# optimusride/altro-cpp

Hardware: AMD Instinct MI355X
Metric: trajectories solved/sec (AL-iLQR to tol), unicycle 101 knots, batched (higher is better)
Workload: dtype f64; 1 GPU; BASELINE configs[2]: batch 4096/GPU unicycle kTurn90 (n=3, m=2, 101 knots), goal + control-bound constraints, full AL loop, default SolverOptions; batch_per_gpu=4096, global_batch=4096, knot_points=101, parallelism=instance-sharded x1 (no data-path collective; RCCL all_gather of result records), device=AMD Radeon Graphics, cus=256

## Files before the change

### altro-cpp_amd/csrc/altro_engine.hpp

```cpp
#pragma once

#include <algorithm>
#include <atomic>
#include <chrono>
#include <cmath>
#include <cstdio>
#include <cstdlib>
#include <cstring>
#include <limits>
#include <map>
#include <string>
#include <thread>
#include <type_traits>
#include <vector>

#include "altro_kernels.hpp"
#include "altro_problem.hpp"

namespace altro_hip {

#define ALTRO_HIP_CHECK(expr)                                                                  \
  do {                                                                                         \
    hipError_t e_ = (expr);                                                                    \
    if (e_ != hipSuccess) {                                                                    \
// ... 1 lines not shown
      snprintf(buf_, sizeof(buf_), "%s:%d: %s -> %s", __FILE__, __LINE__, #expr,               \
               hipGetErrorString(e_));                                                         \
      err_ = buf_;                                                                             \
      return ALTRO_HIP_ERROR;                                                                  \
    }                                                                                          \
  } while (0)

#define ALTRO_TRY(expr)                  \
  do {                                   \
    altro_status st_ = (expr);           \
    if (st_ != ALTRO_OK) return st_;     \
  } while (0)

constexpr int kSpecAuto = -1;
enum FwdSrcSwitch { kFwdSrcAuto = -1, kFwdSrcOther = 0, kFwdSrcGlobal = 1 };
struct Switches {
  struct OptInt {
    bool set = false;
    int v = 0;
  };
  bool poison_on = false;
  unsigned poison_pattern = 0;
  int poison_mix = 0;
  OptInt persist_at;
  bool twin = true;
  bool segments = true;
  OptInt chains;
  OptInt fwd_per_wave;
  int fwd_src = kFwdSrcAuto;
  int sweep_loop = -1;
  OptInt loop_per_cu;
  int cand_front = 6;
  bool twin_debug = false;
  int twin_depth = kTwinDefaultDepth;
  int twin_misclaim = 0;
  const char* sweep_log = nullptr;
  bool loop_log = false;
  bool force_valu_backward = false, force_coop_backward = false;
  bool dense_expansions = true;
  int spec_mode = kSpecAuto;
  bool fast_forward = false;
  bool begin_merged = true;
  bool no_fused = false;

  static bool NotZero(const char* e) { return !(e && atoi(e) == 0); }
  static bool Is(const char* e, const char* what) { return e && std::strcmp(e, what) == 0; }
  Switches() {
    auto env = [](const char* name) { return std::getenv(name); };
    auto number = [&](const char* name) {
      const char* e = env(name);
      return e ? OptInt{true, atoi(e)} : OptInt{};
    };
    if (const char* e = env("ALTRO_HIP_DEBUG_POISON")) {
      poison_on = true;
      poison_pattern = (unsigned)strtoul(e, nullptr, 16);
      poison_mix = std::strchr(e, ',') != nullptr;
    }
    persist_at = number("ALTRO_HIP_PERSIST_AT");
    twin = NotZero(env("ALTRO_HIP_TWIN"));
    segments = NotZero(env("ALTRO_HIP_SEGMENTS"));
    chains = number("ALTRO_HIP_CHAINS");
    if (chains.set) chains.v = std::max(1, std::min(kMaxSweepChains, chains.v));
    fwd_per_wave = number("ALTRO_HIP_FWD_PER_WAVE");
    if (const char* e = env("ALTRO_HIP_FWD_SRC")) fwd_src = Is(e, "global") ? kFwdSrcGlobal : kFwdSrcOther;
    if (const char* e = env("ALTRO_HIP_SWEEP_LOOP")) sweep_loop = NotZero(e) ? 1 : 0;
    loop_per_cu = number("ALTRO_HIP_LOOP_PER_CU");
    if (const char* e = env("ALTRO_HIP_CAND_FRONT")) cand_front = std::max(0, std::min(kLineSearchLanes - 1, atoi(e)));
    twin_debug = env("ALTRO_HIP_TWIN_DEBUG") != nullptr;
    if (const char* e = env("ALTRO_HIP_TWIN_DEPTH")) twin_depth = std::max(1, std::min(kTwinMaxDepth, atoi(e)));
    if (const char* e = env("ALTRO_HIP_TWIN_MISCLAIM")) twin_misclaim = std::max(0, atoi(e));
    sweep_log = env("ALTRO_HIP_SWEEP_LOG");
    loop_log = env("ALTRO_HIP_LOOP_LOG") != nullptr;
    force_valu_backward = Is(env("ALTRO_HIP_BACKWARD"), "valu");
    force_coop_backward = Is(env("ALTRO_HIP_BACKWARD"), "coop");
    dense_expansions = env("ALTRO_HIP_NO_DENSE_EXPANSIONS") == nullptr;
    const char* spec = env("ALTRO_HIP_SPECULATION");
    spec_mode = Is(spec, "off") ? (int)kSpecOff : Is(spec, "free") ? (int)kSpecFree : Is(spec, "wave") ? (int)kSpecWave : kSpecAuto;
    fast_forward = env("ALTRO_HIP_FAST_FORWARD_STALLS") != nullptr;
    begin_merged = !Is(env("ALTRO_HIP_BEGIN_SOLVE"), "split");
    no_fused = env("ALTRO_HIP_NO_FUSED_SWEEP") != nullptr;
  }
};

inline DevOpts ToDevOpts(const altro_options& o) {
  DevOpts d{};
  d.max_iterations_total = o.max_iterations_total;
  d.max_iterations_outer = o.max_iterations_outer;
  d.max_iterations_inner = o.max_iterations_inner;
  d.bp_reg_fail_threshold = o.bp_reg_fail_threshold;
  d.check_forwardpass_bounds = o.check_forwardpass_bounds;
  d.line_search_max_iterations = o.line_search_max_iterations;
  d.reset_duals = o.reset_duals;
  d.cost_tolerance = o.cost_tolerance;
  d.gradient_tolerance = o.gradient_tolerance;
  d.bp_reg_increase_factor = o.bp_reg_increase_factor;
  d.bp_reg_initial = o.bp_reg_initial;
  d.bp_reg_max = o.bp_reg_max;
  d.bp_reg_min = o.bp_reg_min;
  d.state_max = o.state_max;
  d.control_max = o.control_max;
  d.line_search_lower_bound = o.line_search_lower_bound;
  d.line_search_upper_bound = o.line_search_upper_bound;
// ... 1401 lines not shown
  altro_status SetTrajectoryImpl(const ProblemSpec& s) {
    if (!uploaded_) return ALTRO_OK;
    ALTRO_HIP_CHECK(hipSetDevice(desc_.device_id));
    ALTRO_TRY(Sync());
    const double* Xh = !s.has_X ? nullptr : (s.X_view ? s.X_view : s.X.data());
    const double* Uh = !s.has_U ? nullptr : (s.U_view ? s.U_view : s.U.data());
    ALTRO_TRY(UploadRec(A_.X, N_ + 1, R::nP, n, Xh, s.traj_per_instance != 0));
    ALTRO_TRY(UploadRec(A_.U, N_, R::mP, m, Uh, s.traj_per_instance != 0));
    ALTRO_HIP_CHECK(CopySync(X_init_, A_.X, (size_t)(N_ + 1) * R::nP * Bp_ * sizeof(T), hipMemcpyDeviceToDevice));
    ALTRO_HIP_CHECK(CopySync(U_init_, A_.U, (size_t)N_ * R::mP * Bp_ * sizeof(T), hipMemcpyDeviceToDevice));
    return ALTRO_OK;
  }

  altro_status CheckKnotModels(const ProblemSpec& s) {
    for (size_t k = 0; k < s.knot_model.size() && (int)k < desc_.N; ++k) {
      const int w = s.knot_model[k];
      if (w < 0 || w >= kModelCount) {
        err_ = "altro_set_knot_models: knot " + std::to_string(k) + " asks for model " + std::to_string(w) + ", this handle's model " +
               (kModelCount > 1 ? "source lists " + std::to_string(kModelCount) + " models (ALTRO_USER_MODELS)"
                                : std::string("is a single model (a user source with #define ALTRO_USER_MODELS A, B, ... holds several)"));
        return ALTRO_INVALID_ARG;
      }
    }
    return ALTRO_OK;
  }
  size_t ExpBytes(size_t columns) const { return ((size_t)kBwdFrontPad + (size_t)N_ + 2) * RR::EP * columns * sizeof(RS); }
  void SizeShadowColumns() {
    B_ = desc_.batch;
    N_ = desc_.N;
    Bp_ = ((B_ + kBlock - 1) / kBlock) * kBlock;
    twin_cap_ = 0;
    if constexpr (kMfmaBackward) {
      if (sw_.twin && !sw_.fast_forward && !sw_.no_fused) {
        const int want = std::min({Bp_, 16384, ((persist_at_ * 3 / 2 + 8 + kBlock - 1) / kBlock) * kBlock});
        if (ExpBytes((size_t)(Bp_ + want)) < (size_t)0xffffffffu) twin_cap_ = want;
      }
    }
    seg_total_ = 0;
    seg_col0_ = Bp_;
    if constexpr (kMfmaBackward) {
      if (sw_.segments && !sw_.fast_forward && B_ > persist_at_) {
        const int want = (Bp_ * 5 / 8) / kBlock * kBlock;
        if (ExpBytes((size_t)(Bp_ + want + twin_cap_)) < (size_t)0xffffffffu) seg_total_ = want;
      }
    }
    seg_parts_ = 4;
    Bp_ += seg_total_ + twin_cap_;
  }
  static UserTypeTable UserTypes() {
    UserTypeTable t;
    for (int i = 0; i < UserCostList::size; ++i) t.cost_nparams.push_back(UserCostParams(i));
    for (int i = 0; i < UserConList::size; ++i) {
      int np = -1, p = -1, eq = -1;
      UserConInfo(i, &np, &p, &eq);
      t.con_nparams.push_back(np);
      t.con_p.push_back(p);
      t.con_eq.push_back(eq);
    }
    return t;
  }
  altro_status AdoptProblem(const CompiledProblem<T>& cp) {
    if (cp.status != ALTRO_OK) {
      err_ = cp.err;
      return cp.status;
    }
    pd_ = cp.pd;
    knot_class_ = cp.knot_class;
// ... 820 lines not shown
        A.act_list = d_loop_tail_;
        A.act_count = d_loop_ctl_ + kLwTail;
      } else if (whole_batch) {
        A.act_list = nullptr;
        A.act_count = nullptr;
        A.act_count_const = B_;
      } else if (lists.n == 1) {
        A.act_list = lists.list[0];
        A.act_count = lists.count[0];
      } else {
        int* const merged_count = d_counter_ + (size_t)C * r.cstride;
        hipLaunchKernelGGL((k_merge_lists<0>), dim3(1), dim3(256), 0, stream_, lists, d_merged_, merged_count);
        A.act_list = d_merged_;
        A.act_count = merged_count;
        timing_.launches += 1;
      }
      A.host_count = nullptr;
      A.next_list = nullptr;
      A.next_count = nullptr;
      PoisonLds();
      if (r.prof) {
        r.fused_ev = r.nev;
        hipEventRecord(ProfEvent(r.nev++), stream_);
      }
      bool circles = false;
      for (int k = 0; k < pd_.nruns; ++k)
        circles = circles || pd_.runs[k].fast == kFastC || pd_.runs[k].fast == kFastCB || pd_.runs[k].fast == kFastBC;
      int* const out = r.loop_launched ? d_loop_ctl_ + kLwWords : d_counter_ + r.max_sweeps + 2;
      const int spec = sw_.spec_mode == kSpecAuto ? (circles ? (int)kSpecWave : (int)kSpecFree) : sw_.spec_mode;
      TwinCtl tw{};
      if (twin_cap_ > 0 && !A.hist && !r.d.fast_forward_stalls) {
        if (!twin_box_clean_)
          hipMemsetAsync(d_twin_box_, 0, TwinBoxWords() * sizeof(unsigned long long), stream_);
        const int pool = std::min(twin_cap_, std::max(ninst, num_cus_ - ninst));
        tw = TwinCtl{d_twin_box_, d_twin_box_ + (size_t)2 * twin_cap_ * kTwWords, ninst, twin_cap_, Bp_ - twin_cap_, kTwinLag, sw_.twin_debug ? 1 : 0,
                     pool, any_split ? 1 : sw_.twin_depth, sw_.twin_misclaim};
      }
      const dim3 g(ninst + (tw.base > 0 ? tw.npool : 0)), b3(kFwdWaves * kBlock), b4((kFwdWaves + 1) * kBlock);
      timing_.twin_workgroups = tw.base > 0 ? (int)g.x - ninst : 0;
      ForEachFusedVariant([&](auto v) {
        using V = decltype(v);
        if (V::circles == circles && V::spec == spec && V::segments == any_split)
          hipLaunchKernelGGL((k_sweep_fused<T, M, V::circles, V::spec, V::segments>), g, V::spec == kSpecOff ? b3 : b4, fused_lds_bytes_,
                             stream_, A, d_pd_, pd_, r.d, r.mode, 1, out, tw);
      });
      if (r.prof) hipEventRecord(ProfEvent(r.nev++), stream_);
      r.persistent_launched = true;
      timing_.launches += 1;
    }
    return ALTRO_OK;
  }
  altro_status WaitForDevice(SolveRun& r) {
    if (r.nap_ok && !r.nap)
      r.nap = r.loop_launched || std::chrono::duration<double, std::micro>(std::chrono::steady_clock::now() - r.t0).count() > kHostNapAfterUs;
    if (r.nap && tail_ev_) {
      ALTRO_HIP_CHECK(hipEventRecord(tail_ev_, stream_));
      for (;;) {
        const hipError_t q = hipEventQuery(tail_ev_);
        if (q == hipSuccess) break;
        if (q != hipErrorNotReady) ALTRO_HIP_CHECK(q);
        std::this_thread::sleep_for(std::chrono::microseconds(20));
        timing_.host_naps += 1;
      }
    }
    for (int c = 1; c < r.C; ++c) ALTRO_HIP_CHECK(hipStreamSynchronize(r.chain[c].st));
    ALTRO_HIP_CHECK(hipStreamSynchronize(stream_));
    ALTRO_HIP_CHECK(hipGetLastError());
    return ALTRO_OK;
  }
// ... 45 lines not shown
      }
      if (twin_cap_ > 0 && sw_.twin_debug) ALTRO_TRY(DumpTwinMailboxes());
      if (extra[kRwSyncErr] != 0) {
        err_ = "k_sweep_fused: a forward wave gave up waiting for its sequence word (software synchronisation)";
        return ALTRO_HIP_ERROR;
      }
      timing_.fused_sweeps = extra[kRwChainLoops];
      timing_.fused_instance_iterations = extra[kRwUnits];
      sweeps = std::max(sweeps, extra[kRwSweeps]);
    }
    timing_.sweeps = sweeps;
    return ALTRO_OK;
  }
  size_t TwinBoxWords() const { return (size_t)2 * twin_cap_ * (kTwWords + 1); }
  altro_status DumpTwinMailboxes() {
    const int nbox = 2 * twin_cap_;
    std::vector<unsigned long long> box((size_t)nbox * kTwWords);
    ALTRO_HIP_CHECK(CopySync(box.data(), d_twin_box_, box.size() * sizeof(unsigned long long), hipMemcpyDeviceToHost));
    int hist[4] = {0, 0, 0, 0}, why[8] = {0}, by_depth[kTwinMaxDepth + 2] = {0};
    unsigned long long t0 = ~0ull;
    for (int s = 0; s < twin_cap_; ++s)
      if (box[(size_t)s * kTwWords + kTwStamp + kTsPStart]) t0 = std::min(t0, box[(size_t)s * kTwWords + kTwStamp + kTsPStart]);
    auto us_of = [&](const unsigned long long* ts, int i) { return ts[i] ? (double)(long long)(ts[i] - t0) * 0.01 : -1.0; };
    int shown = 0;
    double last_commit = 0, last_pend = 0, last_tstart = 0, last_leave = 0;
    int s_commit = -1, s_pend = -1;
    for (int s = 0; s < nbox; ++s) {
      const unsigned long long* w = &box[(size_t)s * kTwWords];
      const unsigned long long* ts = w + kTwStamp;
      auto us = [&](int i) { return us_of(ts, i); };
      if (s >= twin_cap_ && w[kTwClaim] != 0) {
        hist[w[kTwHand] & 3]++;
        by_depth[std::min<unsigned long long>(w[kTwGen], kTwinMaxDepth + 1)]++;
        const int limit = timing_.twin_claims <= 48 ? 1 : 8;
        if ((shown++ % limit) == 0)
          fprintf(stderr, "  segment %4d depth %d inst %d from %d: it %d..%d hand %d | start %.0f go %.0f cloned %.0f first %.0f snap %.0f claimed %.0f "
                  "done %.0f (loops %llu) verdict %.0f handed %.0f commit %.0f\n", s, (int)w[kTwGen], (int)w[kTwInst] - 1, (int)w[kTwPred] - 1,
                  (int)(w[kTwClaim] >> 32), (int)w[kTwEnd], (int)(w[kTwHand] & 3), us(kTsTStart), us(kTsTGo), us(kTsTCloned), us(kTsTFirst), us(kTsPSnap),
                  us(kTsPClaim), us(kTsTDone), ts[kTsTLoops], us(kTsTVerdict), us(kTsPHand), us(kTsTCommit));
      }
      if (w[kTwWhy] != 0) {
        why[w[kTwWhy] & 7]++;
        if (why[w[kTwWhy] & 7] <= 3)
          fprintf(stderr, "  worker %d refused its successor: why %d at it_inner %d (claim start %d)\n", s, (int)(w[kTwWhy] & 7),
                  (int)((w[kTwWhy] >> 8) & 0xffff), (int)((w[kTwWhy] >> 24) & 0xffff));
      }
      if (us(kTsTCommit) > last_commit) { last_commit = us(kTsTCommit); s_commit = s; }
      if (us(kTsPEnd) > last_pend) { last_pend = us(kTsPEnd); s_pend = s; }
      last_leave = std::max(last_leave, us(kTsPHand));
      last_tstart = std::max(last_tstart, us(kTsTStart));
    }
    fprintf(stderr, "twin timeline: last commit %.0f us (mailbox %d), last primary that finished by itself %.0f us (slot %d), last hand-over %.0f us, "
            "last pool start %.0f us\n", last_commit, s_commit, last_pend, s_pend, last_leave, last_tstart);
    fprintf(stderr, "twin mailboxes: pool %d claims %d confirmed joints %d | segments by depth: 1: %d 2: %d 3: %d 4: %d 5: %d | hand word: open %d ok %d refused %d "
            "revoked %d | refusals: streak broke %d, passed %d, counters %d, rho %d, drho %d, break since snapshot %d\n", (int)timing_.twin_workgroups,
            (int)timing_.twin_claims, (int)timing_.twin_handovers, by_depth[1], by_depth[2], by_depth[3], by_depth[4], by_depth[5], hist[0], hist[1], hist[2],
            hist[3], why[1], why[2], why[3], why[4], why[5], why[6]);
    return ALTRO_OK;
  }
  void AccountProfile(SolveRun& r) {
    float ms = 0, fused_ms = 0;
    hipEventElapsedTime(&ms, prof_ev_[0], prof_ev_[1]);
    timing_.init_ms = ms;
    for (int c = 0; c < r.C; ++c) {
      const std::vector<size_t>& ev = r.chain[c].ev;
      for (size_t e0 = 0; e0 + 3 < ev.size(); e0 += 3) {
        hipEventElapsedTime(&ms, prof_ev_[ev[e0]], prof_ev_[ev[e0 + 1]]);
        timing_.expansions_ms += ms;
        hipEventElapsedTime(&ms, prof_ev_[ev[e0 + 1]], prof_ev_[ev[e0 + 2]]);
        timing_.backward_pass_ms += ms;
        hipEventElapsedTime(&ms, prof_ev_[ev[e0 + 2]], prof_ev_[ev[e0 + 3]]);
        timing_.forward_pass_ms += ms;
      }
// ... 154 lines not shown
```

### altro-cpp_amd/csrc/altro_kernels.hpp

```cpp
#pragma once

#include <type_traits>

#include "altro_device.hpp"

namespace altro_hip {

constexpr int kFwdWaves = 3;
constexpr int kEAheadToErrWord = -7;
constexpr int kFwdSpinLimit = 1 << 22;
template <int kDummy>
__global__ __launch_bounds__(256) void k_poison_columns(unsigned* arr, unsigned rows, unsigned Bp, unsigned col0, unsigned ncols,
                                                         unsigned words, unsigned pattern, int mix) {
  const size_t per_row = (size_t)ncols * words, total = (size_t)rows * per_row;
  for (size_t i = (size_t)blockIdx.x * 256 + threadIdx.x; i < total; i += (size_t)gridDim.x * 256) {
    const size_t r = i / per_row, w = i - r * per_row;
    arr[(r * Bp + col0) * words + w] = mix ? (pattern ^ ((unsigned)i * 2654435761u)) : pattern;
  }
}
template <int kDummy>
__global__ __launch_bounds__(256) void k_poison_lds(unsigned pattern, int words, int mix, int* sink) {
  extern __shared__ unsigned poison_smem[];
  for (int i = threadIdx.x; i < words; i += 256) poison_smem[i] = mix ? (pattern ^ ((unsigned)i * 2654435761u)) : pattern;
  __syncthreads();
// ... 3202 lines not shown
      load_rec<T, R::nP>(sX + k * R::nP, xr);
#pragma unroll
      for (int i = 0; i < R::mP; ++i) ur[i] = T(0);
      if (k < N) load_rec<T, R::mP>(sU + k * R::mP, ur);
      T E[R::EP];
#pragma unroll
      for (int e = 0; e < R::EP; ++e) E[e] = T(0);
      const T J = knot_cost_expansion<T, n, m>(C, pd, kc, rb, xr, ur, E + R::oLx, E + R::oLu, E + R::oLxx, E + R::oLxu,
                                               E + R::oLuu);
      A.costs[(unsigned)k * Bp + (unsigned)b] = J;
      sCost[k] = J;
      if (k < N) discrete_jacobian<T, M>(xr, ur, T(pd->hstep), E + R::oAB);
      using RS = rec_scalar_t<T, M>;
      using RR = Rec<RS, n, m>;
      store_rec_as<T, RS, R::EP, RR::EP, R::eE>(RECP((RS*)A.EXP, k, RR::EP), E);
    }
    toff = (toff + ((cnt + kBlock - 1) / kBlock) * kBlock) % nthreads;
  }
}

enum SpecMode { kSpecOff = 0, kSpecWave = 1, kSpecFree = 3 };
ALTRO_DEV constexpr bool spec_has_wave4(int spec) { return spec == kSpecWave || spec == kSpecFree; }

struct TwinCtl {
  unsigned long long* box;
  unsigned long long* state;
  int base;
  int cap;
  int col0;
  int lag;
  int debug;
  int npool;
  int depth;
  int misclaim;
};
enum TwinStamp { kTsPStart = 0, kTsPSnap = 1, kTsPClaim = 2, kTsPHand = 3, kTsPLoopsAtSnap = 4, kTsTStart = 5, kTsTGo = 6, kTsTCloned = 7,
                 kTsTFirst = 8, kTsTDone = 9, kTsTVerdict = 10, kTsTCommit = 11, kTsTLoops = 12, kTsPEnd = 13 };
enum TwinWord {
  kTwSeq = 0,
  kTwSnap = 1,
  kTwProg = 7,
  kTwSucc = 8,
  kTwEnd = 9,
  kTwGen = 10,
  kTwInst = 11,
  kTwClaim = 12,
  kTwClaimRho = 13,
  kTwClaimDrho = 14,
  kTwClaimSnap = 15,
  kTwHand = 16,
  kTwHandLoops = 17,
  kTwWhy = 18,
  kTwPred = 19,
  kTwStamp = 20,
  kTwWords = 40
};
constexpr unsigned long long kTwOk = 1, kTwRefused = 2, kTwRevoked = 3;
constexpr unsigned long long kTwSuccId = 0xffffull;
constexpr unsigned long long kTwFrozen = 1ull << 32;
constexpr unsigned long long kTwsSnap = 1, kTwsClosed = 2, kTwsLocked = 4, kTwsFull = 8, kTwsBusy = 16;
#ifndef ALTRO_TWIN_DEPTH
#define ALTRO_TWIN_DEPTH 3
#endif
constexpr int kTwinDefaultDepth = ALTRO_TWIN_DEPTH;
constexpr int kTwinMaxDepth = 5;
constexpr int kTwinMinRemaining = 12;
#ifndef ALTRO_TWIN_LAG
#define ALTRO_TWIN_LAG 1
#endif
constexpr int kTwinLag = ALTRO_TWIN_LAG;
constexpr int kTwinIdlePolls = 1 << 15;
constexpr int kTwinHandPolls = 1 << 16;
ALTRO_DEV unsigned long long tw_load(const unsigned long long* p) {
  return __hip_atomic_load(p, __ATOMIC_RELAXED, __HIP_MEMORY_SCOPE_AGENT);
}
ALTRO_DEV void tw_store(unsigned long long* p, unsigned long long v) {
  __hip_atomic_store(p, v, __ATOMIC_RELAXED, __HIP_MEMORY_SCOPE_AGENT);
}
ALTRO_DEV void tw_order() { asm volatile("s_waitcnt vmcnt(0)" ::: "memory"); }
ALTRO_DEV bool tw_cas(unsigned long long* p, unsigned long long expect, unsigned long long v) {
  return __hip_atomic_compare_exchange_strong(p, &expect, v, __ATOMIC_RELAXED, __ATOMIC_RELAXED, __HIP_MEMORY_SCOPE_AGENT);
}
ALTRO_DEV unsigned long long tw_bits(double x) { return (unsigned long long)__double_as_longlong(x); }
ALTRO_DEV double tw_dbl(unsigned long long x) { return __longlong_as_double((long long)x); }
ALTRO_DEV int tw_remaining(const DevOpts& o, unsigned long long prog, int end_inner) {
  const int it_in = (int)(prog >> 32), it_tot = (int)(prog & 0xffffffffull);
  if (end_inner > 0) return end_inner - it_in;
  const int r1 = o.max_iterations_inner - it_in, r2 = o.max_iterations_total - it_tot;
  return r1 < r2 ? r1 : r2;
}
ALTRO_DEV int tw_keep(int R, int lag) { return (R + lag) / 2 + 1; }
ALTRO_DEV bool tw_claimable(int R, int lag) { return R >= 2 * kTwinMinRemaining && R - tw_keep(R, lag) >= kTwinMinRemaining; }
ALTRO_DEV void tw_cancel_chain(const TwinCtl& tw, unsigned long long* box) {
  unsigned long long nx = __hip_atomic_fetch_or(box + kTwSucc, kTwFrozen, __ATOMIC_RELAXED, __HIP_MEMORY_SCOPE_AGENT) & kTwSuccId;
  for (int guard = 0; nx != 0 && nx <= (unsigned long long)(2 * tw.cap) && guard < (2 << kTwinMaxDepth); ++guard) {
    const int id = (int)nx - 1;
    unsigned long long* sb = tw.box + (size_t)id * kTwWords;
    nx = __hip_atomic_fetch_or(sb + kTwSucc, kTwFrozen, __ATOMIC_RELAXED, __HIP_MEMORY_SCOPE_AGENT) & kTwSuccId;
    tw_cas(sb + kTwHand, 0ull, kTwRefused);
    __hip_atomic_fetch_or(tw.state + id, kTwsClosed, __ATOMIC_RELAXED, __HIP_MEMORY_SCOPE_AGENT);
  }
}

template <class T>
struct TailCtx {
  const DevArrays<T>& A;
  const ProblemDesc* pd;
  const DevOpts& o;
  const TwinCtl& tw;
  int* sweeps_out;
  double* ff;
  int tid;
};
struct TwinWorker {
  unsigned long long* box = nullptr;
  int slot = -1;
  bool is_twin = false;
  int streak = 0;
  int break_total = -1;
  unsigned long long ver = 0;
  bool closed = false;
  bool shown = false;
  unsigned long long succ = 0, claim = 0;
  unsigned long long peek = 0;
  bool full = false;
  bool confirmed = false;
  int loops0 = 0;
  ALTRO_DEV void stamp(const TwinCtl& tw, int which, long long value = -1) const {
    if (box && tw.debug) tw_store(box + kTwStamp + which, (unsigned long long)(value >= 0 ? value : wall_clock64()));
  }
  ALTRO_DEV void close(const TwinCtl& tw) const {
    __hip_atomic_fetch_or(tw.state + slot, kTwsClosed, __ATOMIC_RELAXED, __HIP_MEMORY_SCOPE_AGENT);
  }
};

template <class T, bool SEG, bool SOFT>
ALTRO_DEV void fused_report(const TailCtx<T>& C, int b_real, const int* sync_words, int chain_loops, int units, int skipped) {
  const DevArrays<T>& A = C.A;
  int* const sweeps_out = C.sweeps_out;
  if (sweeps_out && C.tid == 0) {
    atomicMax(sweeps_out + kRwChainLoops, chain_loops);
    atomicAdd(sweeps_out + kRwUnits, units);
    atomicMax(sweeps_out + kRwGroupLoops, units + skipped);
    int chain = 0;
    if (A.chain_size) {
      chain = (SEG && A.seg_end && b_real >= A.B && A.seg_hi > 0 && b_real >= A.seg_lo) ? (b_real - A.seg_lo) / A.seg_hi : b_real / A.chain_size;
      chain = chain < kMaxSweepChains - 1 ? chain : kMaxSweepChains - 1;
    }
    atomicMax(sweeps_out + kRwSweeps, A.chain_base[chain] + chain_loops);
    if (SOFT && sync_words[kSyErr] != 0) atomicMax(sweeps_out + kRwSyncErr, 1);
  }
}

ALTRO_DEV int tw_scan(const TwinCtl& tw, const DevOpts& o, int nsl, int nall, int self, int lane, int* waiting_out) {
  int waiting = 0, key = 0;
  for (int v0 = 0; v0 < nall; v0 += kBlock) {
    const int v = v0 + lane;
    bool open = false;
    if (v < nall) {
      const int id = v < nsl ? v : tw.cap + (v - nsl);
      const unsigned long long st = id == self ? kTwsClosed : tw_load(tw.state + id);
      open = (st & (kTwsClosed | kTwsFull)) == 0 && (v < nsl || (st & kTwsBusy) != 0);
      if (open && (st & kTwsSnap) != 0) {
        const unsigned long long* bx = tw.box + (size_t)id * kTwWords;
        const int R = tw_remaining(o, tw_load(bx + kTwProg), (int)tw_load(bx + kTwEnd));
        open = tw_claimable(R, tw.lag);
        if (open && (st & kTwsLocked) == 0) {
          const int k2 = ((R < 0x7fff ? R : 0x7fff) << 16) | (0xffff - (v & 0xffff));
          key = k2 > key ? k2 : key;
        }
      }
    }
    waiting += __popcll(__ballot(open));
  }
  for (int d = 32; d > 0; d >>= 1) {
    const int other = __shfl_xor(key, d);
    key = other > key ? other : key;
  }
  *waiting_out = waiting;
  return key;
}
template <class T>
ALTRO_DEV int tw_try_claim(const TailCtx<T>& C, int v, int nsl, int self) {
  const TwinCtl& tw = C.tw;
  const DevOpts& o = C.o;
  int* const sweeps_out = C.sweeps_out;
  double* const ff = C.ff;
  int got = 0;
  const int id = v < nsl ? v : tw.cap + (v - nsl);
  unsigned long long* bx = tw.box + (size_t)id * kTwWords;
  const unsigned long long st0 = kTwsSnap | (v < nsl ? 0ull : kTwsBusy);
  if (!tw_cas(tw.state + id, st0, st0 | kTwsLocked)) return 0;
  unsigned long long more = 0;
  const unsigned long long ver = tw_load(bx + kTwSeq);
  if (ver != 0) {
    const unsigned long long* buf = bx + kTwSnap + 3 * (ver & 1);
    const unsigned long long c0 = tw_load(buf), rb = tw_load(buf + 1), db = tw_load(buf + 2);
    const unsigned long long pr = tw_load(bx + kTwProg), so = tw_load(bx + kTwSucc), inst = tw_load(bx + kTwInst);
    const int end_in = (int)tw_load(bx + kTwEnd), gen = (int)((so >> 16) & 0xffffull);
    const bool stable = tw_load(bx + kTwSeq) == ver;
    const int in0 = (int)(c0 >> 32), tot0 = (int)(c0 & 0xffffffffull), in1 = (int)(pr >> 32), tot1 = (int)(pr & 0xffffffffull);
    const int R = tw_remaining(o, pr, end_in);
    if (gen >= tw.depth) more = kTwsFull;
    if (stable && more == 0 && (so & kTwFrozen) == 0 && inst != 0 && in1 >= in0 && in1 - in0 == tot1 - tot0 && tw_claimable(R, tw.lag)) {
      const int ahead = tw_keep(R, tw.lag);
      double rho = tw_dbl(rb), drho = tw_dbl(db);
      for (int jj = 0; jj < in1 - in0 + ahead; ++jj) {
        decrease_reg(o, &rho, &drho);
        increase_reg(o, &rho, &drho);
      }
      const int nth = sweeps_out ? atomicAdd(sweeps_out + kRwClaims, 1) + 1 : 1;
      if (tw.misclaim > 0 && nth % tw.misclaim == 0) rho = tw_dbl(tw_bits(rho) ^ 1ull);
      const bool full = gen + 1 >= tw.depth;
      unsigned long long* mine = tw.box + (size_t)self * kTwWords;
      tw_store(mine + kTwClaimRho, tw_bits(rho));
      tw_store(mine + kTwClaimDrho, tw_bits(drho));
      tw_store(mine + kTwClaimSnap, (unsigned long long)(unsigned)tot0);
      tw_store(mine + kTwClaim, ((unsigned long long)(unsigned)(in1 + ahead) << 32) | (unsigned long long)(unsigned)(tot1 + ahead));
      tw_store(mine + kTwInst, inst);
      tw_store(mine + kTwGen, (unsigned long long)(unsigned)(gen + 1));
      tw_store(mine + kTwEnd, (unsigned long long)(unsigned)end_in);
      tw_store(mine + kTwSucc, (so & kTwSuccId) | ((unsigned long long)(unsigned)(gen + 1) << 16));
      tw_store(mine + kTwPred, (unsigned long long)(unsigned)(id + 1));
      tw_store(tw.state + self, kTwsBusy | (full ? kTwsFull : 0ull));
      tw_store(bx + kTwEnd, (unsigned long long)(unsigned)(in1 + ahead));
      tw_order();
      if (tw_cas(bx + kTwSucc, so, (unsigned long long)(unsigned)(self + 1) | ((unsigned long long)(unsigned)(gen + 1) << 16))) {
        ff[kFfClaimItInner] = (double)(in1 + ahead);
        ff[kFfClaimItTotal] = (double)(tot1 + ahead);
        ff[kFfClaimRho] = rho;
        ff[kFfClaimDrho] = drho;
        ff[kFfClaimInst] = (double)((int)inst - 1);
        if (full) more = kTwsFull;
        got = id + 1;
      } else {
        tw_store(tw.state + self, 0ull);
        if (sweeps_out) atomicSub(sweeps_out + kRwClaims, 1);
      }
    }
  }
  if (more != 0) __hip_atomic_fetch_or(tw.state + id, more, __ATOMIC_RELAXED, __HIP_MEMORY_SCOPE_AGENT);
  __hip_atomic_fetch_and(tw.state + id, ~kTwsLocked, __ATOMIC_RELAXED, __HIP_MEMORY_SCOPE_AGENT);
  return got;
}
template <class T>
ALTRO_DEV void tw_find_work(const TailCtx<T>& C, int self, int lane) {
  const TwinCtl& tw = C.tw;
  const int cnt_slots = C.A.act_count ? *C.A.act_count : C.A.act_count_const;
  const int nsl = cnt_slots < tw.cap ? cnt_slots : tw.cap;
  const int nall = nsl + tw.npool;
  int chosen = -1;
  for (int tries = 0; tries < kTwinIdlePolls && chosen < 0; ++tries) {
    int waiting = 0;
    const int key = tw_scan(tw, C.o, nsl, nall, self, lane, &waiting);
    int got = 0;
    if (key != 0 && lane == 0) got = tw_try_claim(C, 0xffff - (key & 0xffff), nsl, self);
    got = __shfl(got, 0);
    if (got > 0) chosen = got - 1;
    if (chosen < 0) {
      if (key == 0 && waiting == 0) break;
      for (int z = 0; z < (key == 0 ? 8 : 1); ++z) __builtin_amdgcn_s_sleep(127);
    }
  }
  if (lane == 0) {
    C.ff[kFfClaimSource] = (double)chosen;
    if (chosen >= 0) __builtin_amdgcn_fence(__ATOMIC_ACQUIRE, "agent");
  }
}
template <class T, class M, bool SEG>
ALTRO_DEV bool tw_enter_clone(const TailCtx<T>& C, TwinWorker& w, int tslot, long long tstart_clock, int nthreads, int* b,
                              int* b_real) {
  const DevArrays<T>& A = C.A;
  const TwinCtl& tw = C.tw;
  double* const ff = C.ff;
  const int tid = C.tid;
  const int src_id = (int)ff[kFfClaimSource];
  if (src_id < 0) return false;
  w.slot = tw.cap + tslot;
  w.box = tw.box + (size_t)w.slot * kTwWords;
  *b_real = (int)ff[kFfClaimInst];
  const int b_src = src_id < tw.cap ? instance_of_slot(A, src_id, 0) : tw.col0 + (src_id - tw.cap);
  if (tid == 0) {
    w.stamp(tw, kTsTStart, tstart_clock);
    w.stamp(tw, kTsTGo);
  }
  const int bT = tw.col0 + tslot;
  copy_column<T, M>(A, C.pd, (unsigned)b_src, (unsigned)bT, kColTwinClone, tid, nthreads);
  if (tid == 0) {
    if (SEG && A.seg_end) {
      A.seg_end[bT] = kSegNoEnd;
      A.seg_next[bT] = -1;
      A.seg_flag[bT] = 0;
      A.seg_streak[bT] = 2;
    }
    A.cost_prev[bT] = A.cost_cur[bT];
    A.it_inner[bT] = (int)ff[kFfClaimItInner];
    A.it_total[bT] = (int)ff[kFfClaimItTotal];
    A.rho_reg[bT] = ff[kFfClaimRho];
    A.drho[bT] = ff[kFfClaimDrho];
  }
  *b = bT;
  __syncthreads();
  if (tid == 0) w.stamp(tw, kTsTCloned);
  if (tid == 0) {
    ff[kFfClaimOpen] = tw_load(w.box + kTwHand) == 0 ? 1.0 : 0.0;
    if (ff[kFfClaimOpen] == 0.0) w.close(tw);
  }
  __syncthreads();
  return ff[kFfClaimOpen] != 0.0;
}

template <class T>
ALTRO_DEV void fused_adopt_spec(const DevArrays<T>& A, int b, T* sKDf, const T* sKD2, int nKD, double* fh, const double* fh2,
                                int tid, int nthreads) {
  for (int i = tid; i < nKD; i += nthreads) sKDf[i] = sKD2[i];
  if (tid == 0) {
    double h[6];
    h[0] = fh2[kFhDV0]; h[1] = fh2[kFhDV1]; h[2] = fh2[kFhRho]; h[3] = fh2[kFhDrho]; h[4] = fh2[kFhRegLog];
    fh[kFhDV0] = h[0];
    fh[kFhDV1] = h[1];
    fh[kFhRho] = h[2];
    fh[kFhDrho] = h[3];
    A.dV0[b] = h[0];
    A.dV1[b] = h[1];
    A.reg_log[b] = h[4];
    A.rho_reg[b] = h[2];
    A.drho[b] = h[3];
  }
}

template <class T, class M, bool WAVE4>
ALTRO_DEV void fused_expand_ahead(const DevArrays<T>& A, const ProblemDesc* pd, const FwdLds<T>& L, T* sm, T* sPool, T* sCost,
                                  T* sCvalAhead, int* sync_words, int b, int wave, int lane, int loops) {
  constexpr int kAhead = WAVE4 ? 3 : 2;
  const int wi = wave == 0 ? 0 : wave - 1;
  const CtxL<T> CA(A, b, sPool, sm + L.nX + L.nU + L.nKD + 2 * L.rowsP(), sm + L.nX + L.nU + L.nKD,
                   sm + L.nX + L.nU + L.nKD + L.rowsP(), sCvalAhead);
  expansion_from_lds<T, M>(A, pd, CA, sm, sm + L.nX, sCost, b, wi * kBlock + lane, kAhead * kBlock);
  if (lane == 0) FwdSync<true>::post(sync_words + kSyEAhead0 + wi, loops);
// ... 18 lines not shown
    const int it_in = A.it_inner[b], it_tot = A.it_total[b];
    int k = o.max_iterations_inner - 1 - it_in;
    const int k2 = o.max_iterations_total - 1 - it_tot;
    k = k < k2 ? k : k2;
    if (k > 0) {
      A.it_inner[b] = it_in + k;
      A.it_total[b] = it_tot + k;
      for (int j = 0; j < k; ++j) hist_push(A, b);
      skipped = k;
    }
    asm volatile("s_waitcnt vmcnt(0)" ::: "memory");
  }
  return skipped;
}

template <class T>
ALTRO_DEV void fused_seg_joint(const TailCtx<T>& C, int b) {
  const DevArrays<T>& A = C.A;
  double* const ff = C.ff;
  const int flag = A.seg_flag[b];
  const int nxt = A.seg_next[b];
  const bool rc = ff[kFfRejected] != 0.0 && ff[kFfInnerDone] == 0.0;
  double leave = 0.0;
  if ((flag & kSegCancelled) || nxt >= 0)
    leave = seg_joint(A, b, flag, nxt, rc, (int)ff[kFfItInner], (int)ff[kFfItTotal], ff[kFfRho], ff[kFfDrho]) ? 1.0 : 0.0;
  if (leave != 0.0) A.phase[b] = 0;
  ff[kFfSegLeave] = leave;
}

template <class T, bool SEG>
ALTRO_DEV void tw_publish(const TailCtx<T>& C, TwinWorker& w, bool rc, int it_in, int it_tot, int loops, int b, int b_real) {
  const TwinCtl& tw = C.tw;
  const double* ff = C.ff;
  if (rc && w.streak >= 2 && !w.full && (!SEG || !C.A.seg_end || C.A.seg_next[b] < 0)) {
    const unsigned long long cnt = ((unsigned long long)(unsigned)it_in << 32) | (unsigned long long)(unsigned)it_tot;
    tw_store(w.box + kTwProg, cnt);
    if (!w.shown) {
      ++w.ver;
      unsigned long long* buf = w.box + kTwSnap + 3 * (w.ver & 1);
      tw_store(buf, cnt);
      tw_store(buf + 1, tw_bits(ff[kFfRho]));
      tw_store(buf + 2, tw_bits(ff[kFfDrho]));
      tw_store(w.box + kTwInst, (unsigned long long)(unsigned)(b_real + 1));
      __builtin_amdgcn_fence(__ATOMIC_RELEASE, "agent");
      tw_order();
      tw_store(w.box + kTwSeq, w.ver);
      tw_order();
      __hip_atomic_fetch_or(tw.state + w.slot, kTwsSnap, __ATOMIC_RELAXED, __HIP_MEMORY_SCOPE_AGENT);
      w.shown = true;
      w.stamp(tw, kTsPSnap);
      w.stamp(tw, kTsPLoopsAtSnap, loops);
    }
  }
  if (!rc && w.shown) {
    __hip_atomic_fetch_and(tw.state + w.slot, ~kTwsSnap, __ATOMIC_RELAXED, __HIP_MEMORY_SCOPE_AGENT);
    tw_store(w.box + kTwSeq, 0ull);
    w.shown = false;
  }
}
ALTRO_DEV void tw_see_claim(const TwinCtl& tw, TwinWorker& w) {
  const unsigned long long sc = w.peek;
  if (sc != w.succ && (sc & kTwFrozen) == 0 && (sc & kTwSuccId) <= (unsigned long long)(2 * tw.cap)) {
    w.succ = sc;
    w.full = (int)((sc >> 16) & 0xffffull) >= tw.depth;
    if ((sc & kTwSuccId) != 0) {
      w.claim = tw_load(tw.box + (size_t)((sc & kTwSuccId) - 1) * kTwWords + kTwClaim);
      w.stamp(tw, kTsPClaim);
    }
  }
}
template <class T>
ALTRO_DEV bool tw_joint(const TailCtx<T>& C, TwinWorker& w, bool rc, int it_in, int it_tot) {
  const TwinCtl& tw = C.tw;
  const double* ff = C.ff;
  const unsigned long long* sb = tw.box + (size_t)((w.succ & kTwSuccId) - 1) * kTwWords;
  const int s_in = (int)(w.claim >> 32), s_tot = (int)(w.claim & 0xffffffffull);
  bool refuse = !rc || it_in > s_in, hand = false;
  int why = !rc ? 1 : (it_in > s_in ? 2 : 0);
  if (!refuse && it_in == s_in) {
    const unsigned long long c_rho = tw_load(sb + kTwClaimRho), c_drho = tw_load(sb + kTwClaimDrho);
    const int c_snap = (int)tw_load(sb + kTwClaimSnap);
    const bool same = it_tot == s_tot && tw_bits(ff[kFfRho]) == c_rho && tw_bits(ff[kFfDrho]) == c_drho && w.break_total < c_snap;
    why = it_tot != s_tot ? 3 : (tw_bits(ff[kFfRho]) != c_rho ? 4 : (tw_bits(ff[kFfDrho]) != c_drho ? 5 : 6));
    if (same && tw_cas(w.box + kTwSucc, w.succ, w.succ | kTwFrozen)) hand = true; else refuse = true;
    if (same && refuse) why = 2;
// ... 152 lines not shown
  const ProblemDesc* pd = &pd_arg;
  const int tid = threadIdx.x, wave = tid >> 6, lane = tid & 63;
  if (blockIdx.x == 0 && tid == 0) publish_count(A);
  TwinWorker w;
  w.is_twin = tw.base > 0 && (int)blockIdx.x >= tw.base;
  const int tslot = w.is_twin ? (int)blockIdx.x - tw.base : -1;
  w.slot = w.is_twin ? -1 : (int)blockIdx.x;
  int b_real = w.is_twin ? -1 : instance_of_slot(A, w.slot, 0);
  if (!w.is_twin && b_real < 0) return;
  if (w.is_twin && (tslot >= tw.npool || tslot >= tw.cap || !persistent)) return;
  if (!w.is_twin && tw.base > 0 && w.slot < tw.cap && persistent) w.box = tw.box + (size_t)w.slot * kTwWords;
  int b = b_real;
  const int N = A.N;
  const unsigned Bp = A.Bp;
  const FwdLds<T> L{(N + 1) * R::nP, N * R::mP, N * R::KP, pd->total_rows, pd->nslots, R::V};
  const FusedSmem<T> S(smem_raw, L, FusedLds<T>{L, N, nm, pd->npool});
  FwdSpec<T> spec{S.sKD2, L.nKD, S.fh2, S.fh2 + kFhSpecRho, false};
  fused_init_lds(S, o, tid);
  const TailCtx<T> C{A, pd, o, tw, sweeps_out, S.ff, tid};
  bool adopt = false;
  StallWatch stall;
  int skipped = 0;
  int loops = 0;
  bool e_done = false;
#ifdef ALTRO_STAMPS
  if (tid < 32) g_stamp_acc[tid] = 0;
  int spec_iters = 0;
#endif
  const long long tstart_clock = tw.debug ? wall_clock64() : 0;
  if (tid == 0 && !w.is_twin) w.stamp(tw, kTsPStart);
  if (w.is_twin) {
    if (wave == 0) tw_find_work(C, tw.cap + tslot, lane);
    __syncthreads();
    if (!tw_enter_clone<T, M, SEG>(C, w, tslot, tstart_clock, kThreads, &b, &b_real)) return;
  }
  if (wave == 2 && lane == 0) {
    S.ff[kFfInitCost] = A.initial_cost[b];
    S.ff[kFfNeedInitCost] = A.need_init_cost[b] ? 1.0 : 0.0;
  }
  for (;;) {
    const long long st_it = ALTRO_STAMP_T0();
    if (w.box && tid == 0 && !w.closed && !w.full && (w.is_twin || w.shown)) w.peek = tw_load(w.box + kTwSucc);
    if (loops == 0) {
      forward2_stage<T, M>(A, pd, L, smem_raw, S.sPool, 1, 0, tid, kThreads, kKdNone, true, -1, b);
      __syncthreads();
    }
    const CtxL<T> CE(A, b, S.sPool, S.sm + L.nX + L.nU + L.nKD + 2 * L.rowsP(), S.sm + L.nX + L.nU + L.nKD,
                     S.sm + L.nX + L.nU + L.nKD + L.rowsP());
    if (!e_done) {
      expansion_from_lds<T, M>(A, pd, CE, S.sm, S.sm + L.nX, S.sCost, b, tid, kThreads);
      if (adopt) ALTRO_STAMP_ADD(17 + wave, st_it);
      if (SPEC && adopt) lds_barrier(); else __syncthreads();
    }
    if (wave == 0 && adopt) ALTRO_STAMP_ADD(9, st_it);
    const long long st_b = ALTRO_STAMP_T0();

    const bool armed = SPEC != kSpecOff && loops > 0 && S.ff[kFfRejected] != 0.0;
    if (SPEC && adopt) {
      const long long st_cp = ALTRO_STAMP_T0();
      fused_adopt_spec(A, b, S.sKDf, S.sKD2, L.nKD, S.fh, S.fh2, tid, kThreads);
      if (wave == 0) ALTRO_STAMP_ADD(16, st_cp);
    } else if (wave == 0) {
      backward_mfma_body<T, M, false, true>(A, o, 0, lane, blockIdx.x, nullptr, S.sKDf, S.fused_junk, S.fh, 0.0, 0.0, nullptr, b, loops == 0);
    }
    if (SPEC && adopt) lds_barrier(); else __syncthreads();
    if (wave == 0 && adopt) ALTRO_STAMP_ADD(10, st_b);
    const long long st_f = ALTRO_STAMP_T0();
// ... 875 lines not shown
```

### altro-cpp_amd/csrc/inst_unicycle_f64.hip

```cpp
#include "altro_engine.hpp"
namespace altro_hip {
EngineBase* MakeEngineUnicycleF64(const altro_desc& d, std::string* err) { return MakeEngineImpl<double, UnicycleM>(d, err); }
}
```

Before: 669,700 trajectories/s.

## Tune twin work-stealing: lower min share, spread claims, let clones republish

Idle twin workgroups can now split work off primaries that have fewer remaining iterations. The minimum claimable share drops from 12 to 4 by default, while segmented mode keeps 12. The scan key now hashes the slot and worker so that idle workers spread across candidates instead of all choosing the same one, and bucketing by R>>spread evens out the ranking. Cloned workers republish their own snapshot right away, so work can be split again down the chain, and the twin pool is sized to at least the CU count even for small batches. Finer splits add claim and copy overhead and contention on the atomics, and they can also cost extra redundant iterations.

```diff
diff --git a/altro-cpp_amd/csrc/altro_engine.hpp b/altro-cpp_amd/csrc/altro_engine.hpp
--- a/altro-cpp_amd/csrc/altro_engine.hpp
+++ b/altro-cpp_amd/csrc/altro_engine.hpp
@@ -57,7 +57,10 @@
   OptInt loop_per_cu;
   int cand_front = 6;
   bool twin_debug = false;
+  bool twin_debug_all = false;
   int twin_depth = kTwinDefaultDepth;
+  int twin_min = tw_min_share(kTwinDefaultMin);
+  int twin_spread = kTwinDefaultSpread;
   int twin_misclaim = 0;
   const char* sweep_log = nullptr;
   bool loop_log = false;
@@ -92,7 +95,10 @@
     loop_per_cu = number("ALTRO_HIP_LOOP_PER_CU");
     if (const char* e = env("ALTRO_HIP_CAND_FRONT")) cand_front = std::max(0, std::min(kLineSearchLanes - 1, atoi(e)));
     twin_debug = env("ALTRO_HIP_TWIN_DEBUG") != nullptr;
+    twin_debug_all = Is(env("ALTRO_HIP_TWIN_DEBUG"), "all");
     if (const char* e = env("ALTRO_HIP_TWIN_DEPTH")) twin_depth = std::max(1, std::min(kTwinMaxDepth, atoi(e)));
+    if (const char* e = env("ALTRO_HIP_TWIN_MIN")) twin_min = tw_min_share(atoi(e));
+    if (const char* e = env("ALTRO_HIP_TWIN_SPREAD")) twin_spread = std::max(0, std::min(kTwinMaxSpread, atoi(e)));
     if (const char* e = env("ALTRO_HIP_TWIN_MISCLAIM")) twin_misclaim = std::max(0, atoi(e));
     sweep_log = env("ALTRO_HIP_SWEEP_LOG");
     loop_log = env("ALTRO_HIP_LOOP_LOG") != nullptr;
@@ -1560,7 +1566,8 @@
     twin_cap_ = 0;
     if constexpr (kMfmaBackward) {
       if (sw_.twin && !sw_.fast_forward && !sw_.no_fused) {
-        const int want = std::min({Bp_, 16384, ((persist_at_ * 3 / 2 + 8 + kBlock - 1) / kBlock) * kBlock});
+        const int per_cu = ((num_cus_ + kBlock - 1) / kBlock) * kBlock;
+        const int want = std::min({std::max(Bp_, per_cu), 16384, ((persist_at_ * 3 / 2 + 8 + kBlock - 1) / kBlock) * kBlock});
         if (ExpBytes((size_t)(Bp_ + want)) < (size_t)0xffffffffu) twin_cap_ = want;
       }
     }
@@ -2447,9 +2454,10 @@
       if (twin_cap_ > 0 && !A.hist && !r.d.fast_forward_stalls) {
         if (!twin_box_clean_)
           hipMemsetAsync(d_twin_box_, 0, TwinBoxWords() * sizeof(unsigned long long), stream_);
+        const int min_share = any_split ? std::max(sw_.twin_min, kTwinSegMin) : sw_.twin_min;
         const int pool = std::min(twin_cap_, std::max(ninst, num_cus_ - ninst));
         tw = TwinCtl{d_twin_box_, d_twin_box_ + (size_t)2 * twin_cap_ * kTwWords, ninst, twin_cap_, Bp_ - twin_cap_, kTwinLag, sw_.twin_debug ? 1 : 0,
-                     pool, any_split ? 1 : sw_.twin_depth, sw_.twin_misclaim};
+                     pool, any_split ? 1 : sw_.twin_depth, min_share, sw_.twin_spread, sw_.twin_misclaim};
       }
       const dim3 g(ninst + (tw.base > 0 ? tw.npool : 0)), b3(kFwdWaves * kBlock), b4((kFwdWaves + 1) * kBlock);
       timing_.twin_workgroups = tw.base > 0 ? (int)g.x - ninst : 0;
@@ -2561,13 +2569,18 @@
       if (s >= twin_cap_ && w[kTwClaim] != 0) {
         hist[w[kTwHand] & 3]++;
         by_depth[std::min<unsigned long long>(w[kTwGen], kTwinMaxDepth + 1)]++;
-        const int limit = timing_.twin_claims <= 48 ? 1 : 8;
+        const int limit = timing_.twin_claims <= 48 || sw_.twin_debug_all ? 1 : 8;
         if ((shown++ % limit) == 0)
           fprintf(stderr, "  segment %4d depth %d inst %d from %d: it %d..%d hand %d | start %.0f go %.0f cloned %.0f first %.0f snap %.0f claimed %.0f "
                   "done %.0f (loops %llu) verdict %.0f handed %.0f commit %.0f\n", s, (int)w[kTwGen], (int)w[kTwInst] - 1, (int)w[kTwPred] - 1,
                   (int)(w[kTwClaim] >> 32), (int)w[kTwEnd], (int)(w[kTwHand] & 3), us(kTsTStart), us(kTsTGo), us(kTsTCloned), us(kTsTFirst), us(kTsPSnap),
                   us(kTsPClaim), us(kTsTDone), ts[kTsTLoops], us(kTsTVerdict), us(kTsPHand), us(kTsTCommit));
       }
+      if (sw_.twin_debug_all && s < twin_cap_ && ts[kTsPStart] != 0)
+        fprintf(stderr, "  primary %4d: start %.0f snap %.0f claimed %.0f handed %.0f end %.0f\n", s, us(kTsPStart), us(kTsPSnap), us(kTsPClaim),
+                us(kTsPHand), us(kTsPEnd));
+      if (sw_.twin_debug_all && s >= twin_cap_ && w[kTwClaim] == 0 && ts[kTsTIdleEnd] != 0)
+        fprintf(stderr, "  idle %4d: start %.0f left %.0f\n", s, us(kTsTStart), us(kTsTIdleEnd));
       if (w[kTwWhy] != 0) {
         why[w[kTwWhy] & 7]++;
         if (why[w[kTwWhy] & 7] <= 3)
diff --git a/altro-cpp_amd/csrc/altro_kernels.hpp b/altro-cpp_amd/csrc/altro_kernels.hpp
--- a/altro-cpp_amd/csrc/altro_kernels.hpp
+++ b/altro-cpp_amd/csrc/altro_kernels.hpp
@@ -3258,10 +3258,13 @@
   int debug;
   int npool;
   int depth;
+  int min_share;
+  int spread;
   int misclaim;
 };
 enum TwinStamp { kTsPStart = 0, kTsPSnap = 1, kTsPClaim = 2, kTsPHand = 3, kTsPLoopsAtSnap = 4, kTsTStart = 5, kTsTGo = 6, kTsTCloned = 7,
-                 kTsTFirst = 8, kTsTDone = 9, kTsTVerdict = 10, kTsTCommit = 11, kTsTLoops = 12, kTsPEnd = 13 };
+                 kTsTFirst = 8, kTsTDone = 9, kTsTVerdict = 10, kTsTCommit = 11, kTsTLoops = 12, kTsPEnd = 13,
+                 kTsTIdleEnd = 14  };
 enum TwinWord {
   kTwSeq = 0,
   kTwSnap = 1,
@@ -3290,7 +3293,21 @@
 #endif
 constexpr int kTwinDefaultDepth = ALTRO_TWIN_DEPTH;
 constexpr int kTwinMaxDepth = 5;
-constexpr int kTwinMinRemaining = 12;
+#ifndef ALTRO_TWIN_MIN
+#define ALTRO_TWIN_MIN 4
+#endif
+constexpr int kTwinDefaultMin = ALTRO_TWIN_MIN;
+constexpr int kTwinSegMin = 12;
+#ifndef ALTRO_TWIN_SPREAD
+#define ALTRO_TWIN_SPREAD 3
+#endif
+constexpr int kTwinDefaultSpread = ALTRO_TWIN_SPREAD;
+constexpr int kTwinMaxSpread = 14;
+constexpr int kTwinSeeClaim = 3;
+constexpr int kTwinMinFloor = 3;
+constexpr int kTwinMinCeil = 1 << 14;
+ALTRO_HD int tw_min_share(int asked) { return asked < kTwinMinFloor ? kTwinMinFloor : (asked > kTwinMinCeil ? kTwinMinCeil : asked); }
+static_assert(kTwinMinFloor + 1 > kTwinSeeClaim, "tw_keep() of the smallest claimable segment must let the publisher see the claim");
 #ifndef ALTRO_TWIN_LAG
 #define ALTRO_TWIN_LAG 1
 #endif
@@ -3315,8 +3332,8 @@
   const int r1 = o.max_iterations_inner - it_in, r2 = o.max_iterations_total - it_tot;
   return r1 < r2 ? r1 : r2;
 }
-ALTRO_DEV int tw_keep(int R, int lag) { return (R + lag) / 2 + 1; }
-ALTRO_DEV bool tw_claimable(int R, int lag) { return R >= 2 * kTwinMinRemaining && R - tw_keep(R, lag) >= kTwinMinRemaining; }
+ALTRO_HD int tw_keep(int R, int lag) { return (R + lag) / 2 + 1; }
+ALTRO_HD bool tw_claimable(int R, int lag, int min_share) { return R >= 2 * min_share && R - tw_keep(R, lag) >= min_share; }
 ALTRO_DEV void tw_cancel_chain(const TwinCtl& tw, unsigned long long* box) {
   unsigned long long nx = __hip_atomic_fetch_or(box + kTwSucc, kTwFrozen, __ATOMIC_RELAXED, __HIP_MEMORY_SCOPE_AGENT) & kTwSuccId;
   for (int guard = 0; nx != 0 && nx <= (unsigned long long)(2 * tw.cap) && guard < (2 << kTwinMaxDepth); ++guard) {
@@ -3378,8 +3395,9 @@
   }
 }
 
-ALTRO_DEV int tw_scan(const TwinCtl& tw, const DevOpts& o, int nsl, int nall, int self, int lane, int* waiting_out) {
-  int waiting = 0, key = 0;
+ALTRO_DEV unsigned long long tw_scan(const TwinCtl& tw, const DevOpts& o, int nsl, int nall, int self, int lane, int* waiting_out) {
+  int waiting = 0;
+  unsigned long long key = 0;
   for (int v0 = 0; v0 < nall; v0 += kBlock) {
     const int v = v0 + lane;
     bool open = false;
@@ -3390,9 +3408,11 @@
       if (open && (st & kTwsSnap) != 0) {
         const unsigned long long* bx = tw.box + (size_t)id * kTwWords;
         const int R = tw_remaining(o, tw_load(bx + kTwProg), (int)tw_load(bx + kTwEnd));
-        open = tw_claimable(R, tw.lag);
+        open = tw_claimable(R, tw.lag, tw.min_share);
         if (open && (st & kTwsLocked) == 0) {
-          const int k2 = ((R < 0x7fff ? R : 0x7fff) << 16) | (0xffff - (v & 0xffff));
+          const unsigned mix = tw.spread > 0 ? (((unsigned)v * 0x9E3779B1u) ^ ((unsigned)self * 0x85EBCA6Bu)) >> 16 : 0xffffu - (unsigned)v;
+          const unsigned long long k2 = ((unsigned long long)(((R < 0x7fff ? R : 0x7fff) >> tw.spread) + 1) << 32) |
+                                        ((unsigned long long)(mix & 0xffffu) << 16) | (unsigned long long)(v & 0xffff);
           key = k2 > key ? k2 : key;
         }
       }
@@ -3400,7 +3420,7 @@
     waiting += __popcll(__ballot(open));
   }
   for (int d = 32; d > 0; d >>= 1) {
-    const int other = __shfl_xor(key, d);
+    const unsigned long long other = __shfl_xor(key, d);
     key = other > key ? other : key;
   }
   *waiting_out = waiting;
@@ -3428,7 +3448,7 @@
     const int in0 = (int)(c0 >> 32), tot0 = (int)(c0 & 0xffffffffull), in1 = (int)(pr >> 32), tot1 = (int)(pr & 0xffffffffull);
     const int R = tw_remaining(o, pr, end_in);
     if (gen >= tw.depth) more = kTwsFull;
-    if (stable && more == 0 && (so & kTwFrozen) == 0 && inst != 0 && in1 >= in0 && in1 - in0 == tot1 - tot0 && tw_claimable(R, tw.lag)) {
+    if (stable && more == 0 && (so & kTwFrozen) == 0 && inst != 0 && in1 >= in0 && in1 - in0 == tot1 - tot0 && tw_claimable(R, tw.lag, tw.min_share)) {
       const int ahead = tw_keep(R, tw.lag);
       double rho = tw_dbl(rb), drho = tw_dbl(db);
       for (int jj = 0; jj < in1 - in0 + ahead; ++jj) {
@@ -3478,9 +3498,9 @@
   int chosen = -1;
   for (int tries = 0; tries < kTwinIdlePolls && chosen < 0; ++tries) {
     int waiting = 0;
-    const int key = tw_scan(tw, C.o, nsl, nall, self, lane, &waiting);
+    const unsigned long long key = tw_scan(tw, C.o, nsl, nall, self, lane, &waiting);
     int got = 0;
-    if (key != 0 && lane == 0) got = tw_try_claim(C, 0xffff - (key & 0xffff), nsl, self);
+    if (key != 0 && lane == 0) got = tw_try_claim(C, (int)(key & 0xffffull), nsl, self);
     got = __shfl(got, 0);
     if (got > 0) chosen = got - 1;
     if (chosen < 0) {
@@ -3492,6 +3512,22 @@
     C.ff[kFfClaimSource] = (double)chosen;
     if (chosen >= 0) __builtin_amdgcn_fence(__ATOMIC_ACQUIRE, "agent");
   }
+}
+ALTRO_DEV void tw_show(const TwinCtl& tw, TwinWorker& w, unsigned long long cnt, double rho, double drho, int b_real, int loops) {
+  ++w.ver;
+  unsigned long long* buf = w.box + kTwSnap + 3 * (w.ver & 1);
+  tw_store(buf, cnt);
+  tw_store(buf + 1, tw_bits(rho));
+  tw_store(buf + 2, tw_bits(drho));
+  tw_store(w.box + kTwInst, (unsigned long long)(unsigned)(b_real + 1));
+  __builtin_amdgcn_fence(__ATOMIC_RELEASE, "agent");
+  tw_order();
+  tw_store(w.box + kTwSeq, w.ver);
+  tw_order();
+  __hip_atomic_fetch_or(tw.state + w.slot, kTwsSnap, __ATOMIC_RELAXED, __HIP_MEMORY_SCOPE_AGENT);
+  w.shown = true;
+  w.stamp(tw, kTsPSnap);
+  w.stamp(tw, kTsPLoopsAtSnap, loops);
 }
 template <class T, class M, bool SEG>
 ALTRO_DEV bool tw_enter_clone(const TailCtx<T>& C, TwinWorker& w, int tslot, long long tstart_clock, int nthreads, int* b,
@@ -3531,6 +3567,11 @@
   if (tid == 0) {
     ff[kFfClaimOpen] = tw_load(w.box + kTwHand) == 0 ? 1.0 : 0.0;
     if (ff[kFfClaimOpen] == 0.0) w.close(tw);
+    else if ((int)((tw_load(w.box + kTwSucc) >> 16) & 0xffffull) < tw.depth) {
+      const unsigned long long cnt = ((unsigned long long)(unsigned)(int)ff[kFfClaimItInner] << 32) | (unsigned long long)(unsigned)(int)ff[kFfClaimItTotal];
+      tw_store(w.box + kTwProg, cnt);
+      tw_show(tw, w, cnt, ff[kFfClaimRho], ff[kFfClaimDrho], *b_real, 0);
+    }
   }
   __syncthreads();
   return ff[kFfClaimOpen] != 0.0;
@@ -3615,25 +3656,10 @@
 ALTRO_DEV void tw_publish(const TailCtx<T>& C, TwinWorker& w, bool rc, int it_in, int it_tot, int loops, int b, int b_real) {
   const TwinCtl& tw = C.tw;
   const double* ff = C.ff;
-  if (rc && w.streak >= 2 && !w.full && (!SEG || !C.A.seg_end || C.A.seg_next[b] < 0)) {
+  if (rc && (w.streak >= 2 || w.shown) && !w.full && (!SEG || !C.A.seg_end || C.A.seg_next[b] < 0)) {
     const unsigned long long cnt = ((unsigned long long)(unsigned)it_in << 32) | (unsigned long long)(unsigned)it_tot;
     tw_store(w.box + kTwProg, cnt);
-    if (!w.shown) {
-      ++w.ver;
-      unsigned long long* buf = w.box + kTwSnap + 3 * (w.ver & 1);
-      tw_store(buf, cnt);
-      tw_store(buf + 1, tw_bits(ff[kFfRho]));
-      tw_store(buf + 2, tw_bits(ff[kFfDrho]));
-      tw_store(w.box + kTwInst, (unsigned long long)(unsigned)(b_real + 1));
-      __builtin_amdgcn_fence(__ATOMIC_RELEASE, "agent");
-      tw_order();
-      tw_store(w.box + kTwSeq, w.ver);
-      tw_order();
-      __hip_atomic_fetch_or(tw.state + w.slot, kTwsSnap, __ATOMIC_RELAXED, __HIP_MEMORY_SCOPE_AGENT);
-      w.shown = true;
-      w.stamp(tw, kTsPSnap);
-      w.stamp(tw, kTsPLoopsAtSnap, loops);
-    }
+    if (!w.shown) tw_show(tw, w, cnt, ff[kFfRho], ff[kFfDrho], b_real, loops);
   }
   if (!rc && w.shown) {
     __hip_atomic_fetch_and(tw.state + w.slot, ~kTwsSnap, __ATOMIC_RELAXED, __HIP_MEMORY_SCOPE_AGENT);
@@ -3852,7 +3878,14 @@
   if (w.is_twin) {
     if (wave == 0) tw_find_work(C, tw.cap + tslot, lane);
     __syncthreads();
-    if (!tw_enter_clone<T, M, SEG>(C, w, tslot, tstart_clock, kThreads, &b, &b_real)) return;
+    if (!tw_enter_clone<T, M, SEG>(C, w, tslot, tstart_clock, kThreads, &b, &b_real)) {
+      if (tid == 0 && tw.debug) {
+        unsigned long long* own = tw.box + (size_t)(tw.cap + tslot) * kTwWords + kTwStamp;
+        tw_store(own + kTsTStart, (unsigned long long)tstart_clock);
+        tw_store(own + kTsTIdleEnd, (unsigned long long)wall_clock64());
+      }
+      return;
+    }
   }
   if (wave == 2 && lane == 0) {
     S.ff[kFfInitCost] = A.initial_cost[b];
diff --git a/altro-cpp_amd/csrc/inst_unicycle_f64.hip b/altro-cpp_amd/csrc/inst_unicycle_f64.hip
--- a/altro-cpp_amd/csrc/inst_unicycle_f64.hip
+++ b/altro-cpp_amd/csrc/inst_unicycle_f64.hip
@@ -2,3 +2,11 @@
 namespace altro_hip {
 EngineBase* MakeEngineUnicycleF64(const altro_desc& d, std::string* err) { return MakeEngineImpl<double, UnicycleM>(d, err); }
 }
+
+extern "C" int altro_twin_policy(int R, int lag, int asked_min, int* keep, int* claimable, int* see_claim) {
+  const int min_share = altro_hip::tw_min_share(asked_min);
+  if (keep) *keep = altro_hip::tw_keep(R, lag);
+  if (claimable) *claimable = altro_hip::tw_claimable(R, lag, min_share) ? 1 : 0;
+  if (see_claim) *see_claim = altro_hip::kTwinSeeClaim;
+  return min_share;
+}
```

New measurement: 687,800 trajectories/s (median of 6 runs). 1.03x the previous value.
